# yhenon/pixeltable-yolox

Hardware: AMD Instinct MI355X
Metric: images/sec (fwd+NMS) YOLOX-s 640×640 bf16 @1/2/4/8 MI355X; box mAP parity (higher is better)
Workload: dtype bf16

## Files before the change

### pixeltable-yolox_amd/csrc/conv_ws.hip

```cpp
#include "conv_common.hpp"
#include "lds_dma.hpp"

#ifndef YXH_WS_PROBE
#define YXH_WS_PROBE 0
#endif

#ifndef YXH_WS_PD8
#define YXH_WS_PD8 0
#endif

#ifndef YXH_WS_NPIN
#define YXH_WS_NPIN 48
#endif

#ifndef YXH_WS_ACT_CT
#define YXH_WS_ACT_CT 1
#endif

namespace yxh {

namespace {

template <typename T, int CR>
__device__ __forceinline__ uint4 ws_weight_padk(const ConvParams& p, int n_first, int tap, int kb, int lane) {
    const int frow = lane & 15, fq = lane >> 4;
    const int ch = kb * 32 + fq * 8;
    if (ch >= CR) return make_uint4(0, 0, 0, 0);
    const int n = min(n_first + frow, p.cout - 1);
    return *(const uint4*)((const T*)p.w + ((long long)n * 9 + tap) * CR + ch);
}

__device__ __forceinline__ void pin_agpr(uint4& v) {
    typedef unsigned u32x4v __attribute__((ext_vector_type(4)));
    u32x4v t = {v.x, v.y, v.z, v.w};
    asm volatile("" : "+a"(t));
    v = make_uint4(t.x, t.y, t.z, t.w);
}

constexpr int ws_ps(int c16, int s) {
    return s == 1 ? c16 + (6 - c16 % 4) % 4 : (c16 % 2 ? c16 : c16 + 1);
}
constexpr int ws_hxp(int tx, int s) {
    const int hx = (tx - 1) * s + 3;
    if (tx % 16 == 0) return hx;
    int h = hx;
    while (h % 8 != tx % 8) ++h;
    return h;
}

}

template <typename T, int CIN, int S, int TX, int TY, int TN, int WN, int WK, int WM, int BPC, bool F1, int PGN = 0,
          int PGC = 0, int PGH = 0, int CR = CIN, bool A32 = false>
__global__ __launch_bounds__(64 * WN * WK * WM, BPC) void conv_ws(ConvParams p, int tiles_x, int tiles_y,
                                                                 int ntiles, int ntn, int nwork) {
    static_assert(sizeof(T) == 2, "16-bit operands");
    constexpr int NW = WN * WK * WM;
    constexpr int NCB = CIN / 32, WCB = NCB / WK;
    constexpr int WTN = TN / WN, FR = WTN / 16;
    constexpr int TM = TX * TY, WTM = TM / WM, FC = WTM / 16;
    constexpr int HX = (TX - 1) * S + 3, HY = (TY - 1) * S + 3, HXP = ws_hxp(TX, S);
    constexpr int C16 = CIN / 8, PS = ws_ps(C16, S), PSB = PS * 16;
    constexpr int SLOTS = HY * HXP * PS, LOADS = (SLOTS + 63) / 64, GB = (LOADS + NW - 1) / NW;
    constexpr int RBYTES = WK > 1 ? WN * WM * FR * FC * (WK - 1) * 1024 : 0;
    constexpr bool PG = PGN > 0, HP = PGH > 0, PGY = PG || HP;
    constexpr int RS = TN / 8 + 1, RSLOTS = (S == 1 || PGY) ? TM * RS : 0;
    constexpr int RLOADS = (RSLOTS + 63) / 64, GR = (RLOADS + NW - 1) / NW, RTB = RLOADS * 1024;
    constexpr int NRING = 3;
    constexpr int XS = PGC / 8 + 1, XSLOTS = PG && PGC > 0 ? TM * XS : 0;
    constexpr int XLOADS = (XSLOTS + 63) / 64, GX = (XLOADS + NW - 1) / NW, XTB = XLOADS * 1024;
    constexpr int K2 = TN + PGC, KB2 = K2 / 32;
    constexpr int WN2 = PG ? (NW < PGN / 16 ? NW : PGN / 16) : 1, WM2 = NW / WN2;
    constexpr int NF2 = PG ? PGN / 16 / WN2 : 1, PF2 = TM / 16 / WM2;
    static_assert(!PG || (!F1 && TN % 32 == 0 && PGC % 32 == 0 && PGN % (16 * WN2) == 0 &&
                          NW % WN2 == 0 && (TM / 16) % WM2 == 0), "post-conv tile");
    static_assert(!HP || (!PG && !F1 && S == 1 && TN % 32 == 0), "head-form tile");
    constexpr int HROWS = HP ? PGH * 16 : 0, HBYTES_W = HROWS * RS * 16 + HROWS * 4;
    constexpr int NG = CIN / 32, R1 = NW / NG, NPA = (HY * HXP + 15) / 16;
    constexpr int HBYTES = LOADS * 1024;
    constexpr int XOFF = 2 * HBYTES + RBYTES + NRING * RTB;
    constexpr int TOFF = XOFF + 3 * XTB;
    constexpr int HWOFF = TOFF + (F1 ? HBYTES : 0);
    constexpr int SMEM = HWOFF + HBYTES_W;
    static_assert(!F1 || (S == 1 && NW % NG == 0), "fused Bottleneck tile");
    constexpr int FCO = (FC + WK - 1) / WK;
    constexpr int NS = WCB * 9;
    constexpr int PD = YXH_WS_PD8 && FR * FC >= 8 ? YXH_WS_PD8 : FR * FC >= 8 ? 1 : FR * FC >= 4 ? 2 : 3;
    static_assert(NCB % WK == 0 && WTN % 16 == 0 && WTM % 16 == 0 && TM % (16 * WM) == 0, "tile");
    static_assert(FR * 9 * WCB * 4 <= (NW == 4 && BPC == 1 ? 288 : 160), "weights must stay in VGPRs");
    static_assert(SMEM <= 160 * 1024 && SMEM * BPC <= 160 * 1024, "LDS (BPC blocks per CU must fit)");
    constexpr int NPIN = !F1 && FR * 9 * WCB * 4 > 160 ? YXH_WS_NPIN : 0;
    __shared__ __attribute__((aligned(16))) char smem[SMEM];

    const int tid = threadIdx.x, lane = tid & 63;
    const int wave = __builtin_amdgcn_readfirstlane(tid >> 6);
    const int wn = wave % WN, wk = (wave / WN) % WK, wm = wave / (WN * WK);
    const int frow = lane & 15, fq = lane >> 4;
    const int bid = dma::xcd_remap(blockIdx.x, gridDim.x);
    const int nt = bid % ntn, worker = bid / ntn;
    const int n0 = nt * TN;
    const int tile = worker;
    if (tile >= ntiles) return;

    const int cin_ = p.cin, cout = p.cout, in_w = p.in_w, in_h = p.in_h, scs = p.scs[0];
    const int OH = p.out_h, OW = p.out_w, ohw = p.ohw;
    (void)cin_;

    uint32_t boff[FC];
#pragma unroll
    for (int j = 0; j < FC; ++j) {
        const int pl = (wm * FC + j) * 16 + frow;
        const int ty = pl / TX, tx = pl - ty * TX;
        boff[j] = (uint32_t)((ty * S * HXP + tx * S) * PSB + (wk * WCB * 4 + fq) * 16);
    }

    const uint32_t lds0 = dma::lds_addr(smem);
    const uint32_t bytes = (uint32_t)((long long)in_h * in_w * scs * 2);
    const int gsrc = p.grp2 && n0 >= cout / 2 ? CR : 0;

    int hrel[GB], hyx[GB];
#pragma unroll
    for (int i = 0; i < GB; ++i) {
        const int L = wave + NW * i;
        const int s = 64 * L + lane;
        const int hp = s / PS, c16 = s - hp * PS;
        const int hy = hp / HXP, hx = hp - hy * HXP;
        const bool st = L < LOADS && s < SLOTS && c16 < CR / 8 && hx < HX;
        hyx[i] = st ? (hy | (hx << 16)) : 0x7fff7fff;
        hrel[i] = ((hy * in_w + hx) * scs + c16 * 8) * 2;
    }

    struct TileC { int b, oy0, ox0; };
    const unsigned txy = (unsigned)(tiles_x * tiles_y);
    auto coords = [&](int t) -> TileC {
        const unsigned b = (unsigned)t / txy, r = (unsigned)t - b * txy;
        const unsigned ty = r / (unsigned)tiles_x, tx = r - ty * (unsigned)tiles_x;
        return TileC{(int)b, (int)ty * TY, (int)tx * TX};
    };

    auto issue_halo = [&](const TileC& c, int kb) {
        const int iy0 = c.oy0 * S - 1, ix0 = c.ox0 * S - 1;
        const int base = (iy0 * in_w + ix0) * scs * 2;
        const dma::u32x4 rsrc = dma::srd((const T*)p.sptr[0] + (long long)c.b * p.sbs[0] + gsrc, bytes);
#pragma unroll
        for (int i = 0; i < GB; ++i) {
            const int L = wave + NW * i;
            if (LOADS % NW == 0 || i + 1 < GB || L < LOADS) {
                const int iy = iy0 + (hyx[i] & 0xffff), ix = ix0 + (hyx[i] >> 16);
                const bool ok = (unsigned)iy < (unsigned)in_h && (unsigned)ix < (unsigned)in_w;
                const uint32_t voff = ok ? (uint32_t)(base + hrel[i]) : dma::kOob;
                dma::load16(rsrc, voff, 0u, __builtin_amdgcn_readfirstlane(lds0 + (uint32_t)(kb * HBYTES + L * 1024)));
            }
// ... 339 lines not shown
            for (int j = 0; j < FC; ++j) acc[i][j] = f32x4{0.f, 0.f, 0.f, 0.f};
        const char* hb = F1 ? smem + TOFF : smem + kb * HBYTES;
        uint4 bf[PD + 1][FC];
        auto load_b = [&](int s, uint4 (&d)[FC]) {
            const int c = s / 9, tap = s - 9 * (s / 9);
            const int ky = tap / 3, kx = tap - 3 * (tap / 3);
            const int so = (ky * HXP + kx) * PSB + c * 64;
#pragma unroll
            for (int j = 0; j < FC; ++j) d[j] = *(const uint4*)(hb + boff[j] + so);
        };
#pragma unroll
        for (int q = 0; q < PD; ++q)
            if (q < NS) load_b(q, bf[q]);
        __builtin_amdgcn_sched_group_barrier(0x100, FC * (PD < NS ? PD : NS), 0);
        EpiCtx e{};
        if constexpr (EPI) e = epi_ctx(prev, k - 1);
        PostCtx pc{};
        if constexpr (POST) pc = post_ctx(prev2, k - 2);
        uint4 pob[KBP];
#pragma unroll
        for (int s = 0; s < NS; ++s) {
            if (s + PD < NS) load_b(s + PD, bf[(s + PD) % (PD + 1)]);
            const int c = s / 9, tap = s - 9 * (s / 9);
            if constexpr (FIRST && NPIN > 0) {
#pragma unroll
                for (int i = 0; i < FR; ++i)
                    if ((c * 9 + tap) * FR + i < NPIN) pin_agpr(a[i][tap][c]);
            }
            if constexpr (HP) {
#pragma unroll
                for (int i = 0; i < FR; ++i)
#pragma unroll
                    for (int j = 0; j < FC; ++j) Mma<T>::run(acc[i][j], a[i][tap][c], bf[s % (PD + 1)][j]);
            } else {
#pragma unroll
                for (int j = 0; j < FC; ++j)
#pragma unroll
                    for (int i = 0; i < FR; ++i) Mma<T>::run(acc[i][j], a[i][tap][c], bf[s % (PD + 1)][j]);
            }
            if constexpr (EPI)
                if (s < NP) epi_piece(e, accp, s / FR, s % FR, act_c);
            if constexpr (POST && SPLIT) {
                if (s >= 1 && (s - 1) % SP == 0 && (s - 1) / SP < NPU) post_math(pc, (s - 1) / SP, pob);
                if (s % SP == 0 && s / SP < NPU) post_load(pc, s / SP, pob);
            } else if constexpr (POST) {
                if (s % SP == 0 && s / SP < NPU) post_piece(pc, s / SP);
            }
            if (s + PD < NS) __builtin_amdgcn_sched_group_barrier(0x100, FC, 0);
#pragma unroll
            for (int m = 0; m < FR * FC; ++m) {
                __builtin_amdgcn_sched_group_barrier(0x008, 1, 0);
                if constexpr (EPI) __builtin_amdgcn_sched_group_barrier(0x002, 2, 0);
            }
        }
        if constexpr (EPI)
#pragma unroll
            for (int q = NS; q < NP; ++q) epi_piece(e, accp, q / FR, q % FR, act_c);
        if constexpr (POST) {
            if (SPLIT && (NS - 1) % SP == 0 && (NS - 1) / SP < NPU) post_math(pc, (NS - 1) / SP, pob);
#pragma unroll
            for (int u = (NS + SP - 1) / SP; u < NPU; ++u) post_piece(pc, u);
        }

        if constexpr (WK > 1) {
            char* red = smem + 2 * HBYTES;
            const int grp = wm * WN + wn;
#pragma unroll
            for (int i = 0; i < FR; ++i)
#pragma unroll
                for (int j = 0; j < FC; ++j) {
                    const int own = j % WK;
                    if (own != wk) {
                        const int slot = wk < own ? wk : wk - 1;
                        *(f32x4*)(red + (((grp * FR + i) * FC + j) * (WK - 1) + slot) * 1024 + lane * 16) = acc[i][j];
                    }
                }
            dma::barrier();
#pragma unroll
            for (int i = 0; i < FR; ++i)
#pragma unroll
                for (int j = 0; j < FC; ++j)
                    if (j % WK == wk) {
                        f32x4 v = acc[i][j];
#pragma unroll
                        for (int o = 0; o < WK - 1; ++o)
                            v += *(const f32x4*)(red + (((grp * FR + i) * FC + j) * (WK - 1) + o) * 1024 + lane * 16);
                        accp[i][j / WK] = v;
                    }
        } else {
#pragma unroll
            for (int i = 0; i < FR; ++i)
#pragma unroll
                for (int j = 0; j < FC; ++j) accp[i][j] = acc[i][j];
        }
        return next;
    };

    using act_rt = std::integral_constant<int, 0>;
    int next = tile_step(cur, tile, 0, cnext, cur, cur, std::false_type{}, std::false_type{}, std::true_type{}, act_rt{});
    if constexpr (HP) {
        const T* hw = (const T*)(hgrp1 ? p.pgw2 : p.pgw);
        const float* hb = hgrp1 ? p.pgb2 : p.pgb;
        char* wl = smem + HWOFF;
        for (int q = tid; q < HROWS * (TN / 8); q += 64 * NW) {
            const int r = q / (TN / 8), c = q - (TN / 8) * (q / (TN / 8));
            *(uint4*)(wl + (r * RS + c) * 16) = r < hrows ? *(const uint4*)(hw + (long long)r * TN + c * 8)
                                                          : make_uint4(0, 0, 0, 0);
        }
        for (int q = tid; q < HROWS; q += 64 * NW) ((float*)(wl + HROWS * RS * 16))[q] = q < hrows ? hb[q] : 0.0f;
    }

    constexpr bool ACT_CT = YXH_WS_ACT_CT && !A32 && !PGY && !F1 && NW == 4 && BPC == 1;
    if constexpr (ACT_CT) {
        auto tile_loop = [&](auto act_c) {
            int k = 1;
            for (; next < ntiles; ++k) {
                prev2 = prev;
                prev = cur;
                cur = cnext;
                next = tile_step(cur, next, k, cnext, prev, prev2, std::true_type{}, std::false_type{}, std::false_type{},
                                 act_c);
            }
            epilogue(cur, k - 1, accp, act_c);
        };
        if (silu) tile_loop(std::integral_constant<int, 1>{});
        else tile_loop(std::integral_constant<int, 2>{});
    } else {
        int k = 1;
        for (; next < ntiles; ++k) {
            prev2 = prev;
            prev = cur;
            cur = cnext;
            if (PGY && k >= 2)
                next = tile_step(cur, next, k, cnext, prev, prev2, std::true_type{}, std::integral_constant<bool, PGY>{},
                                 std::false_type{}, act_rt{});
            else
                next = tile_step(cur, next, k, cnext, prev, prev2, std::true_type{}, std::false_type{}, std::false_type{},
                                 act_rt{});
        }
        if constexpr (PGY) {
            dma::wait_vm<0>();
            dma::barrier();
            if (k >= 2) post_all(post_ctx(prev, k - 2));
        }
        epilogue(cur, k - 1, accp, act_rt{});
        if constexpr (PGY) {
            dma::barrier();
            post_all(post_ctx(cur, k - 1));
        }
    }
    (void)ohw;
}

template <typename T, int CIN, int S, int TX, int TY, int TN, int WN, int WK, int WM, int BPC = 1, bool F1 = false,
          int PGN = 0, int PGC = 0, int PGH = 0, int CR = CIN, bool A32 = false>
static int launch_ws(const ConvParams& p, hipStream_t st) {
    if (p.stride != S || p.cin != CR) {
        set_error("conv_ws variant built for stride %d, %d input channels", S, CR);
        return YXH_EUNSUPPORTED;
    }
    if (CR != CIN && (p.grp2 || PGN > 0 || PGH > 0 || F1 || p.scs[0] % 8 || (uintptr_t)p.sptr[0] % 16)) {
        set_error("conv_ws padded-K variant (%d -> %d channels): plain conv over 16-byte pixel rows only", CR, CIN);
        return YXH_EUNSUPPORTED;
    }
    if (PGH > 0) {
        if (!p.grp2 || !p.pgw2 || p.cout != 2 * TN || (p.pg_cout + 15) / 16 != PGH) {
            set_error("conv_ws head-form tile: two groups of %d channels, %d class fragments", TN, PGH);
            return YXH_EUNSUPPORTED;
        }
    } else if ((p.pgw != nullptr) != (PGN > 0) || p.pgw2 || (p.pg_store && PGN == 0) ||
               (PGN > 0 && (p.pg_cout != PGN || p.pgs_ch != PGC || p.cout != TN))) {
        set_error(PGN > 0 ? "conv_ws post tile built for %d -> %d channels + a %d-channel post_src, post conv %d"
                          : "conv_ws plain tile with a post conv (%d -> %d, %d, %d)",
                  CIN, TN, PGC, PGN);
        return YXH_EUNSUPPORTED;
    }
    if (p.grp2 && (F1 || PGN > 0 || (p.cout / 2) % TN)) {
        set_error("conv_ws variant (%d input channels) cannot split its channel tiles over two groups", CIN);
        return YXH_EUNSUPPORTED;
    }
    if ((p.pw1 != nullptr) != F1) {
        set_error(F1 ? "conv_ws fused-Bottleneck variant (%d input channels) needs pre_weight"
                     : "conv_ws plain variant (%d input channels) with a pre_weight",
                  CIN);
        return YXH_EUNSUPPORTED;
    }
    if (A32) {
        if (!p.dst_f32 || p.act != YXH_ACT_NONE || p.res || p.grp2 || p.cout % 4 || ((uintptr_t)p.dst % 16) ||
            p.dst_cs % 4 || p.dst_bs % 4 || (long long)p.ohw * p.dst_cs * 4 >= (1LL << 31)) {
            set_error("conv_ws fp32-gradient tile: fp32 dst of 16-byte rows, no activation / residual");
            return YXH_EUNSUPPORTED;
        }
    } else if (p.dst_f32 || p.accum || (p.act != YXH_ACT_SILU && p.act != YXH_ACT_NONE) ||
        (!p.vec_store && PGN == 0 && PGH == 0) ||
        p.cout % 8 || (p.res && (S != 1 || ((uintptr_t)p.res % 16) || p.res_cs % 8 || p.res_bs % 8))) {
        set_error("conv_ws: 16-bit dst, SiLU/no activation, 8-byte aligned dst rows, 16-byte residual rows "
                  "(stride-1 variants) only");
        return YXH_EUNSUPPORTED;
    }
    const int tiles_x = (p.out_w + TX - 1) / TX, tiles_y = (p.out_h + TY - 1) / TY;
    const long long ntiles = (long long)tiles_x * tiles_y * (p.M / p.ohw);
    const int ntn = (p.cout + TN - 1) / TN;
    if (ntiles >= (1LL << 30)) {
        set_error("conv_ws: too many tiles");
        return YXH_EINVAL;
    }
    const int nwork = (int)std::min<long long>(ntiles, std::max(1, p.cus * BPC / ntn));
    hipLaunchKernelGGL((conv_ws<T, CIN, S, TX, TY, TN, WN, WK, WM, BPC, F1, PGN, PGC, PGH, CR, A32>), dim3((unsigned)(nwork * ntn)),
                       dim3(64 * WN * WK * WM), 0, st, p, tiles_x, tiles_y, (int)ntiles, ntn, nwork);
    YXH_CHECK_LAUNCH("conv_ws launch");
    return YXH_OK;
}

template <typename T>
static int ws_dispatch_t(int id, const ConvParams& p, hipStream_t st) {
    switch (id) {
        case 1: return launch_ws<T, 32, 1, 16, 8, 32, 1, 1, 4>(p, st);
        case 2: return launch_ws<T, 32, 1, 16, 16, 32, 1, 1, 8>(p, st);
        case 3: return launch_ws<T, 32, 2, 16, 8, 64, 2, 1, 4>(p, st);
        case 4: return launch_ws<T, 32, 2, 16, 4, 64, 2, 1, 2, 2>(p, st);
        case 5: return launch_ws<T, 64, 1, 16, 8, 64, 2, 1, 4>(p, st);
        case 6: return launch_ws<T, 64, 1, 16, 4, 64, 2, 1, 2, 2>(p, st);
        case 7: return launch_ws<T, 64, 2, 16, 4, 128, 4, 1, 2>(p, st);
        case 8: return launch_ws<T, 64, 2, 16, 2, 128, 4, 1, 1, 2>(p, st);
        case 11: return launch_ws<T, 128, 1, 8, 4, 128, 4, 2, 1>(p, st);
        case 12: return launch_ws<T, 128, 1, 8, 8, 64, 2, 2, 1>(p, st);
        case 13: return launch_ws<T, 128, 2, 16, 2, 128, 4, 2, 1>(p, st);
        case 14: return launch_ws<T, 128, 2, 8, 4, 128, 4, 2, 1>(p, st);
        case 15: return launch_ws<T, 128, 1, 16, 4, 64, 2, 2, 1>(p, st);
        case 16: return launch_ws<T, 256, 1, 8, 4, 64, 2, 4, 1>(p, st);
        case 17: return launch_ws<T, 256, 1, 16, 2, 64, 2, 4, 1>(p, st);
        case 18: return launch_ws<T, 32, 1, 16, 8, 32, 1, 1, 4, 2>(p, st);
        case 19: return launch_ws<T, 64, 1, 32, 2, 64, 2, 1, 2, 2>(p, st);
        case 20: return launch_ws<T, 128, 1, 16, 2, 64, 2, 2, 1, 2>(p, st);
        case 21: return launch_ws<T, 128, 1, 8, 4, 64, 2, 2, 1, 2>(p, st);
        case 22: return launch_ws<T, 128, 2, 16, 1, 64, 2, 2, 1, 2>(p, st);
        case 23: return launch_ws<T, 256, 1, 8, 2, 32, 1, 4, 1, 2>(p, st);
        case 24: return launch_ws<T, 64, 2, 16, 2, 64, 2, 1, 2, 2>(p, st);
        case 25: return launch_ws<T, 128, 1, 16, 4, 128, 4, 1, 1>(p, st);
        case 26: return launch_ws<T, 128, 1, 16, 2, 128, 4, 1, 1>(p, st);
        case 27: return launch_ws<T, 128, 1, 8, 4, 128, 4, 1, 1>(p, st);
        case 28: return launch_ws<T, 256, 2, 8, 2, 32, 1, 4, 1>(p, st);
        case 29: return launch_ws<T, 256, 2, 8, 2, 64, 2, 4, 1>(p, st);
        case 30: return launch_ws<T, 256, 2, 16, 1, 32, 1, 4, 1>(p, st);
        case 31: return launch_ws<T, 32, 1, 16, 8, 32, 1, 1, 4, 1, true>(p, st);
        case 32: return launch_ws<T, 32, 1, 16, 16, 32, 1, 1, 8, 1, true>(p, st);
        case 33: return launch_ws<T, 64, 1, 16, 4, 64, 2, 1, 2, 1, true>(p, st);
        case 34: return launch_ws<T, 64, 1, 16, 8, 64, 2, 1, 2, 1, true>(p, st);
        case 35: return launch_ws<T, 128, 1, 16, 4, 128, 4, 1, 1, 1, true>(p, st);
        case 36: return launch_ws<T, 128, 1, 8, 4, 128, 4, 1, 1, 1, true>(p, st);
        case 41: return launch_ws<T, 32, 1, 16, 8, 32, 1, 1, 4, 1, false, 64, 32>(p, st);
        case 42: return launch_ws<T, 32, 1, 16, 4, 32, 1, 1, 4, 2, false, 64, 32>(p, st);
        case 43: return launch_ws<T, 64, 1, 16, 4, 64, 2, 1, 2, 1, false, 128, 64>(p, st);
        case 44: return launch_ws<T, 64, 1, 8, 4, 64, 2, 2, 1, 2, false, 128, 64>(p, st);
        case 45: return launch_ws<T, 64, 2, 16, 2, 128, 4, 1, 1, 1, false, 128, 0>(p, st);
        case 46: return launch_ws<T, 64, 2, 16, 4, 128, 4, 1, 1, 1, false, 128, 0>(p, st);
        case 47: return launch_ws<T, 64, 1, 16, 2, 64, 2, 2, 1, 2, false, 128, 64>(p, st);
        case 48: return launch_ws<T, 64, 1, 16, 4, 64, 2, 2, 1, 1, false, 128, 64>(p, st);
        case 49: return launch_ws<T, 64, 2, 16, 2, 128, 4, 2, 1, 1, false, 128, 0>(p, st);
        case 50: return launch_ws<T, 64, 2, 8, 4, 128, 4, 2, 1, 1, false, 128, 0>(p, st);
        case 51: return launch_ws<T, 128, 1, 16, 4, 128, 4, 1, 1, 1, false, 0, 0, 5>(p, st);
        case 53: return launch_ws<T, 128, 1, 16, 2, 128, 4, 1, 1, 1, false, 0, 0, 5>(p, st);
        case 52: return launch_ws<T, 64, 1, 16, 8, 64, 2, 1, 2, 1, false, 64, 0>(p, st);
        case 54: return launch_ws<T, 64, 1, 16, 4, 64, 2, 1, 2, 1, false, 64, 0>(p, st);
        case 55: return launch_ws<T, 128, 1, 8, 4, 128, 4, 1, 1, 1, false, 128, 0>(p, st);
        case 56: return launch_ws<T, 128, 1, 16, 2, 128, 4, 1, 1, 1, false, 128, 0>(p, st);
        case 61: return launch_ws<T, 96, 1, 16, 4, 80, 5, 1, 1, 1, false, 0, 0, 0, 80>(p, st);
        case 62: return launch_ws<T, 96, 1, 16, 4, 32, 2, 1, 2, 2, false, 0, 0, 0, 80>(p, st);
        case 63: return launch_ws<T, 96, 2, 16, 4, 80, 5, 1, 1, 1, false, 0, 0, 0, 80>(p, st);
        case 64: return launch_ws<T, 96, 2, 16, 4, 32, 2, 1, 2, 1, false, 0, 0, 0, 80>(p, st);
        case 65: return launch_ws<T, 160, 1, 16, 4, 64, 4, 1, 1>(p, st);
        case 66: return launch_ws<T, 160, 1, 16, 4, 32, 2, 1, 2>(p, st);
        case 67: return launch_ws<T, 160, 2, 16, 2, 64, 4, 1, 1>(p, st);
        case 68: return launch_ws<T, 160, 2, 16, 2, 32, 2, 1, 2>(p, st);
        case 69: return launch_ws<T, 320, 1, 8, 4, 32, 2, 2, 1>(p, st);
        case 71: return launch_ws<T, 320, 1, 16, 2, 32, 2, 2, 1>(p, st);
        case 72: return launch_ws<T, 320, 2, 16, 1, 32, 2, 2, 1>(p, st);
        case 74: return launch_ws<T, 512, 1, 8, 2, 32, 2, 4, 1>(p, st);
        case 76: return launch_ws<T, 512, 1, 16, 1, 32, 2, 4, 1>(p, st);
        case 79: return launch_ws<T, 160, 1, 16, 2, 64, 4, 1, 1>(p, st);
        case 80: return launch_ws<T, 96, 1, 8, 4, 32, 2, 1, 2, 2, false, 0, 0, 0, 80>(p, st);
        case 81: return launch_ws<T, 96, 1, 16, 4, 32, 2, 1, 2, 2, false, 0, 0, 0, 80, true>(p, st);
        case 82: return launch_ws<T, 160, 1, 16, 4, 64, 4, 1, 1, 1, false, 0, 0, 0, 160, true>(p, st);
        case 83: return launch_ws<T, 160, 1, 16, 4, 32, 2, 1, 2, 1, false, 0, 0, 0, 160, true>(p, st);
        case 84: return launch_ws<T, 320, 1, 8, 4, 32, 2, 2, 1, 1, false, 0, 0, 0, 320, true>(p, st);
        case 85: return launch_ws<T, 320, 1, 16, 2, 32, 2, 2, 1, 1, false, 0, 0, 0, 320, true>(p, st);
        case 86: return launch_ws<T, 64, 1, 16, 4, 64, 2, 1, 2, 2, false, 0, 0, 0, 64, true>(p, st);
        case 87: return launch_ws<T, 128, 1, 16, 4, 128, 4, 1, 1, 1, false, 0, 0, 0, 128, true>(p, st);
        case 88: return launch_ws<T, 256, 1, 8, 4, 64, 2, 4, 1, 1, false, 0, 0, 0, 256, true>(p, st);
        case 89: return launch_ws<T, 32, 1, 16, 4, 80, 5, 1, 1, 1, false, 0, 0, 0, 16>(p, st);
        default: set_error("conv_ws tile id %d", id); return YXH_EINVAL;
    }
}

int conv_ws_dispatch(int dtype, int id, const ConvParams& p, hipStream_t st) {
    if (p.taps != 9 || p.kw != 3 || p.pad != 1 || p.nsrc != 1 || p.sup[0] || p.sw[0] != p.in_w) {
        set_error("conv_ws needs a 3x3 pad-1 conv over one plain source");
        return YXH_EUNSUPPORTED;
    }
    if ((long long)p.in_h * p.in_w * p.scs[0] * 2 >= (1LL << 31)) {
        set_error("conv_ws: image exceeds 31-bit byte offsets");
        return YXH_EUNSUPPORTED;
    }
    if (dtype == YXH_BF16) return ws_dispatch_t<bf16>(id, p, st);
    if (dtype == YXH_F16) return ws_dispatch_t<f16>(id, p, st);
    set_error("conv_ws is built for bf16/f16");
    return YXH_EUNSUPPORTED;
}

}
```

### pixeltable-yolox_amd/csrc/conv_ws1.hip

```cpp
#include "conv_common.hpp"
#include "lds_dma.hpp"

namespace yxh {

template <typename T, int CIN, int TM, int TN, int WN, int WK, int WM, int BPC, int NBUF, bool UP0, bool V16>
__global__ __launch_bounds__(64 * WN * WK * WM, BPC) void conv_ws1(ConvParams p, int ntiles, int ntn, int nwork,
                                                                    int ps, int l0, int l1) {
    static_assert(sizeof(T) == 2, "16-bit operands");
    constexpr int NW = WN * WK * WM;
    constexpr int NCB = CIN / 32, WCB = NCB / WK;
    constexpr int WTN = TN / WN, FR = WTN / 16;
    constexpr int WTM = TM / WM, FC = WTM / 16;
    constexpr int C16 = CIN / 8;
    constexpr int LMAX = (TM * (C16 + 6) + 63) / 64 + 2, GB = (LMAX + NW - 1) / NW, HBYTES = GB * NW * 1024;
    constexpr int RBYTES = WK > 1 ? WN * WM * FR * FC * (WK - 1) * 1024 : 0;
    constexpr int SMEM = NBUF * HBYTES + RBYTES;
    static_assert(NBUF >= 2 && (NBUF - 1) * GB <= 63, "DMA pipeline depth");
    constexpr int FCO = (FC + WK - 1) / WK;
    constexpr int PD = FR * FC >= 8 ? 1 : FR * FC >= 4 ? 2 : 3;
    static_assert(NCB % WK == 0 && WTN % 16 == 0 && WTM % 16 == 0, "tile");
    static_assert(FR * WCB * 4 <= (NW == 4 && BPC == 1 ? 288 : 160), "weights must stay in VGPRs");
    static_assert(SMEM <= 160 * 1024, "LDS");
    __shared__ __attribute__((aligned(16))) char smem[SMEM];

    const int tid = threadIdx.x, lane = tid & 63;
    const int wave = __builtin_amdgcn_readfirstlane(tid >> 6);
    const int wn = wave % WN, wk = (wave / WN) % WK, wm = wave / (WN * WK);
    const int frow = lane & 15, fq = lane >> 4;
    const int bid = dma::xcd_remap(blockIdx.x, gridDim.x);
    const int nt = bid % ntn, worker = bid / ntn;
    const int n0 = nt * TN;
    const int tile = worker;
    if (tile >= ntiles) return;
    const int M = p.M, cout = p.cout, dcs = p.dst_cs;
    const int c0 = p.src0_ch, ncb0 = c0 / 32;
    const int c1 = CIN - c0;

    uint32_t boff[FC];
#pragma unroll
    for (int j = 0; j < FC; ++j) boff[j] = (uint32_t)(((wm * FC + j) * 16 + frow) * ps * 16 + fq * 16);

    int geo[GB];
#pragma unroll
    for (int i = 0; i < GB; ++i) {
        const int L = wave + NW * i;
        const int r = L < l0 ? 0 : 1;
        const int s = 64 * (L - r * l0) + lane;
        const int hp = s / ps, ch = s - hp * ps;
        const bool st = L < l0 + l1 && hp < TM && ch < (r ? c1 : c0) / 8;
        geo[i] = st ? (hp | (ch << 16)) : -1;
    }
    const uint32_t lds0 = dma::lds_addr(smem);
    const long long src0_elems = UP0 ? (long long)(M / p.ohw) * p.sbs[0] : (long long)M * p.scs[0];
    const dma::u32x4 srd0 = dma::srd(p.sptr[0], (uint32_t)(src0_elems * 2));
    const int ohw = p.ohw, ow = p.out_w, sw0 = p.sw[0];
    const long long sbs0 = p.sbs[0];
    const dma::u32x4 srd1 = dma::srd(p.nsrc > 1 ? p.sptr[1] : p.sptr[0],
                                     (uint32_t)((long long)M * (p.nsrc > 1 ? p.scs[1] : p.scs[0]) * 2));
    const int scs0 = p.scs[0], scs1 = p.nsrc > 1 ? p.scs[1] : 0;

    auto issue = [&](int t, int kb) {
        const int m0 = t * TM;
#pragma unroll
        for (int i = 0; i < GB; ++i) {
            const int L = wave + NW * i;
            {
                const int g = geo[i];
                const int m = m0 + (g & 0xffff);
                const bool ok = g >= 0 && m < M;
                const uint32_t ldsa = __builtin_amdgcn_readfirstlane(lds0 + (uint32_t)(kb * HBYTES + L * 1024));
                const bool r0 = L < l0;
                dma::u32x4 rs = r0 ? srd0 : srd1;
                rs.x = __builtin_amdgcn_readfirstlane(rs.x);
                rs.y = __builtin_amdgcn_readfirstlane(rs.y);
                rs.z = __builtin_amdgcn_readfirstlane(rs.z);
                rs.w = __builtin_amdgcn_readfirstlane(rs.w);
                long long e = (long long)m * (r0 ? scs0 : scs1);
                if (UP0 && r0) {
                    const int b = m / ohw, rr = m - b * ohw, y = rr / ow, x = rr - y * ow;
                    e = b * sbs0 + ((long long)(y >> 1) * sw0 + (x >> 1)) * scs0;
                }
                const uint32_t voff = ok ? (uint32_t)((e + (g >> 16) * 8) * 2) : dma::kOob;
                dma::load16(rs, voff, 0u, ldsa);
            }
        }
    };

#pragma unroll
    for (int q = 0; q < NBUF; ++q) issue(tile + q * nwork, q);
    uint4 a[FR][WCB];
#pragma unroll
    for (int c = 0; c < WCB; ++c)
#pragma unroll
        for (int i = 0; i < FR; ++i) a[i][c] = ws_weight<T>(p, n0 + wn * WTN + i * 16, 0, 1, CIN, wk * WCB + c, lane);
    float bias[FR][4];
#pragma unroll
    for (int i = 0; i < FR; ++i) {
        const int n = n0 + wn * WTN + i * 16 + fq * 4;
#pragma unroll
        for (int r = 0; r < 4; ++r) bias[i][r] = n + r < cout ? p.bias[n + r] : 0.0f;
    }

    const bool silu = p.act == YXH_ACT_SILU;
    typedef uint32_t u32x2 __attribute__((ext_vector_type(2)));
    const __amdgpu_buffer_rsrc_t dsrd =
        __builtin_amdgcn_make_buffer_rsrc(p.dst, (short)0, (int)((long long)M * dcs * 2), 0x00020000);
    auto epi_piece = [&](const int tprev, const f32x4 (&ap)[FR][FCO], const int o, const int i) {
        const int j = wk + WK * o;
        const int m = tprev * TM + (wm * FC + j) * 16 + frow;
        const int n = n0 + wn * WTN + i * 16 + fq * 4;
        const bool ok = j < FC && m < M && n < cout;
        const int od = ok ? (m * dcs + n) * 2 : (int)dma::kOob;
        const f32x4 x = ap[i][o] + f32x4{bias[i][0], bias[i][1], bias[i][2], bias[i][3]};
        const f32x4 v = silu ? yxh::silu4(x) : x;
        T t[4] = {from_f32<T>(v[0]), from_f32<T>(v[1]), from_f32<T>(v[2]), from_f32<T>(v[3])};
        u32x2 u;
        __builtin_memcpy(&u, t, 8);
        __builtin_amdgcn_raw_buffer_store_b64(u, dsrd, od, 0, 0);
    };

    auto epi_piece16 = [&](const int tprev, const f32x4 (&ap)[FR][FCO], const int o, const int ip) {
        const int j = wk + WK * o;
        const int i0 = 2 * ip;
        const int m = tprev * TM + (wm * FC + j) * 16 + frow;
        const int n = n0 + wn * WTN + i0 * 16 + (fq & 1) * 16 + (fq >> 1) * 8;
        const bool ok = j < FC && m < M && n < cout;
        const int od = ok ? (m * dcs + n) * 2 : (int)dma::kOob;
        uint32_t w[2][2];
#pragma unroll
        for (int h = 0; h < 2; ++h) {
            const int i = i0 + h;
            const f32x4 x = ap[i][o] + f32x4{bias[i][0], bias[i][1], bias[i][2], bias[i][3]};
            const uint2 pk = pack4<T>(silu ? yxh::silu4(x) : x);
            w[h][0] = pk.x;
            w[h][1] = pk.y;
        }
#pragma unroll
        for (int q = 0; q < 2; ++q) {
            const auto r = __builtin_amdgcn_permlane16_swap(w[0][q], w[1][q], false, false);
            w[0][q] = r[0];
            w[1][q] = r[1];
        }
        typedef uint32_t u32x4 __attribute__((ext_vector_type(4)));
        const u32x4 u = {w[0][0], w[0][1], w[1][0], w[1][1]};
        __builtin_amdgcn_raw_buffer_store_b128(u, dsrd, od, 0, 0);
    };

    f32x4 accp[FR][FCO];
    static_assert(!V16 || FR % 2 == 0, "16-byte epilogue pairs channel fragments");
    constexpr int NP = V16 ? FR / 2 * FCO : FR * FCO;
    constexpr int PFR = V16 ? FR / 2 : FR;
    constexpr int PSP = V16 && 2 * NP <= WCB ? 2 : 1;
    auto piece = [&](const int tprev, const f32x4 (&ap)[FR][FCO], const int q) {
        if constexpr (V16) epi_piece16(tprev, ap, q / PFR, q % PFR);
        else epi_piece(tprev, ap, q / FR, q % FR);
    };
    auto tile_step = [&](const int t, const int k, const int tprev, auto epi, auto first) -> int {
        constexpr bool EPI = decltype(epi)::value;
        constexpr bool FIRST = decltype(first)::value;
        const int kb = k % NBUF;
        const int next = t + nwork;
        if constexpr (FIRST) {
            constexpr int younger = (NBUF - 1) * GB + FR * WCB;
            dma::wait_vm<(younger < 63 ? younger : 63)>();
        } else {
            dma::wait_vm<(NBUF - 2) * GB>();
        }
        dma::barrier();
        if (!FIRST) issue(t + (NBUF - 1) * nwork, (k + NBUF - 1) % NBUF);

        f32x4 acc[FR][FC];
#pragma unroll
        for (int i = 0; i < FR; ++i)
#pragma unroll
            for (int j = 0; j < FC; ++j) acc[i][j] = f32x4{0.f, 0.f, 0.f, 0.f};
        const char* hb = smem + kb * HBYTES;
        uint4 bf[PD + 1][FC];
        auto load_b = [&](int s, uint4 (&d)[FC]) {
            const int cg = wk * WCB + s;
            const int so = cg < ncb0 ? cg * 64 : l0 * 1024 + (cg - ncb0) * 64;
#pragma unroll
            for (int j = 0; j < FC; ++j) d[j] = *(const uint4*)(hb + boff[j] + so);
        };
#pragma unroll
        for (int q = 0; q < PD; ++q)
            if (q < WCB) load_b(q, bf[q]);
        __builtin_amdgcn_sched_group_barrier(0x100, FC * (PD < WCB ? PD : WCB), 0);
#pragma unroll
        for (int s = 0; s < WCB; ++s) {
            if (s + PD < WCB) load_b(s + PD, bf[(s + PD) % (PD + 1)]);
#pragma unroll
            for (int j = 0; j < FC; ++j)
#pragma unroll
                for (int i = 0; i < FR; ++i) Mma<T>::run(acc[i][j], a[i][s], bf[s % (PD + 1)][j]);
            if constexpr (EPI)
                if (s % PSP == 0 && s / PSP < NP) piece(tprev, accp, s / PSP);
            if (s + PD < WCB) __builtin_amdgcn_sched_group_barrier(0x100, FC, 0);
#pragma unroll
            for (int m = 0; m < FR * FC; ++m) {
                __builtin_amdgcn_sched_group_barrier(0x008, 1, 0);
                if constexpr (EPI) __builtin_amdgcn_sched_group_barrier(0x002, 2, 0);
            }
        }
        if constexpr (EPI)
#pragma unroll
            for (int q = (WCB + PSP - 1) / PSP; q < NP; ++q) piece(tprev, accp, q);

        if constexpr (WK > 1) {
            char* red = smem + NBUF * HBYTES;
            const int grp = wm * WN + wn;
#pragma unroll
            for (int i = 0; i < FR; ++i)
#pragma unroll
                for (int j = 0; j < FC; ++j) {
                    const int own = j % WK;
                    if (own != wk) {
                        const int slot = wk < own ? wk : wk - 1;
                        *(f32x4*)(red + (((grp * FR + i) * FC + j) * (WK - 1) + slot) * 1024 + lane * 16) = acc[i][j];
                    }
                }
            dma::barrier();
#pragma unroll
            for (int i = 0; i < FR; ++i)
#pragma unroll
                for (int j = 0; j < FC; ++j)
                    if (j % WK == wk) {
                        f32x4 v = acc[i][j];
#pragma unroll
                        for (int o = 0; o < WK - 1; ++o)
                            v += *(const f32x4*)(red + (((grp * FR + i) * FC + j) * (WK - 1) + o) * 1024 + lane * 16);
                        accp[i][j / WK] = v;
                    }
        } else {
#pragma unroll
            for (int i = 0; i < FR; ++i)
#pragma unroll
                for (int j = 0; j < FC; ++j) accp[i][j] = acc[i][j];
        }
        return next;
    };

    int cur = tile;
    int next = tile_step(cur, 0, 0, std::false_type{}, std::true_type{});
    int k = 1;
    for (; next < ntiles; ++k) {
        const int prev = cur;
        cur = next;
        next = tile_step(cur, k, prev, std::true_type{}, std::false_type{});
    }
#pragma unroll
    for (int q = 0; q < NP; ++q) piece(cur, accp, q);
    dma::wait_vm<0>();
}

template <typename T, int CIN, int TM, int TN, int WN, int WK, int WM, int BPC = 1, int NBUF = 2, bool UP0 = false>
static int launch_ws1(const ConvParams& p, hipStream_t st) {
    if (p.cin != CIN) {
        set_error("conv_ws1 variant built for %d input channels", CIN);
        return YXH_EUNSUPPORTED;
    }
    const int c0 = p.src0_ch, c1 = CIN - c0;
    const bool srcs_ok = UP0 ? (p.nsrc == 2 && p.sup[0] == 1 && p.sup[1] == 0 && p.sw[0] * 2 == p.out_w &&
                                p.sw[1] == p.out_w && p.sbs[1] == (long long)p.ohw * p.scs[1] &&
                                (long long)(p.M / p.ohw) * p.sbs[0] * 2 < (1LL << 31))
                             : (bool)p.src_dense;
    if (!srcs_ok || !p.dst_dense || p.dst_f32 || p.accum || p.res || p.pw1 || p.grp2 ||
        (p.act != YXH_ACT_SILU && p.act != YXH_ACT_NONE) || p.cout % 8 || c0 % 32 || c1 % 32 ||
        (p.nsrc == 1) != (c1 == 0)) {
        set_error("conv_ws1: dense 1x1 over 32-channel-aligned sources, 16-bit dst, SiLU/no activation, %d input channels",
                  CIN);
        return YXH_EUNSUPPORTED;
    }
    const long long M = p.M;
    if (M * p.scs[0] * 2 >= (1LL << 31) || (p.nsrc > 1 && M * p.scs[1] * 2 >= (1LL << 31)) ||
        M * p.dst_cs * 2 >= (1LL << 31)) {
        set_error("conv_ws1: tensors exceed 31-bit byte offsets");
        return YXH_EUNSUPPORTED;
    }
    int ps = std::max(c0, c1) / 8;
    ps += (6 - ps % 4) % 4;
    const int l0 = (TM * ps + 63) / 64, l1 = c1 ? (TM * ps + 63) / 64 : 0;
    if (l0 + l1 > (TM * (CIN / 8 + 6) + 63) / 64 + 2) {
        set_error("conv_ws1: source split %d + %d does not fit the LDS image", c0, c1);
        return YXH_EUNSUPPORTED;
    }
    const long long ntiles = (M + TM - 1) / TM;
    const int ntn = (p.cout + TN - 1) / TN;
    const int nwork = (int)std::min<long long>(ntiles, std::max(1, p.cus * BPC / ntn));
    constexpr bool PAIRS = (TN / WN / 16) % 2 == 0;
    if (p.v16_req && !PAIRS) {
        set_error("conv_ws1 tile has no 16-byte epilogue (an odd number of channel fragments per wave)");
        return YXH_EUNSUPPORTED;
    }
    if (PAIRS && p.v16_req && p.vec16)
        hipLaunchKernelGGL((conv_ws1<T, CIN, TM, TN, WN, WK, WM, BPC, NBUF, UP0, PAIRS>), dim3((unsigned)(nwork * ntn)),
                           dim3(64 * WN * WK * WM), 0, st, p, (int)ntiles, ntn, nwork, ps, l0, l1);
    else
        hipLaunchKernelGGL((conv_ws1<T, CIN, TM, TN, WN, WK, WM, BPC, NBUF, UP0, false>), dim3((unsigned)(nwork * ntn)),
                           dim3(64 * WN * WK * WM), 0, st, p, (int)ntiles, ntn, nwork, ps, l0, l1);
    YXH_CHECK_LAUNCH("conv_ws1 launch");
    return YXH_OK;
}

template <typename T>
static int ws1_dispatch_t(int id, const ConvParams& p, hipStream_t st) {
    switch (id) {
        case 1: return launch_ws1<T, 64, 128, 64, 2, 1, 2, 2>(p, st);
        case 2: return launch_ws1<T, 64, 256, 64, 2, 1, 4, 1>(p, st);
        case 3: return launch_ws1<T, 128, 64, 128, 4, 1, 1, 2>(p, st);
        case 4: return launch_ws1<T, 128, 128, 64, 2, 1, 2, 1>(p, st);
        case 5: return launch_ws1<T, 256, 64, 128, 4, 1, 1, 2>(p, st);
        case 6: return launch_ws1<T, 256, 64, 64, 2, 1, 2, 2>(p, st);
        case 7: return launch_ws1<T, 512, 32, 128, 4, 1, 1, 1>(p, st);
        case 8: return launch_ws1<T, 512, 64, 64, 2, 2, 2, 1>(p, st);
        case 9: return launch_ws1<T, 1024, 32, 64, 2, 2, 2, 1>(p, st);
        case 10: return launch_ws1<T, 256, 128, 128, 4, 1, 2, 1>(p, st);
        case 11: return launch_ws1<T, 64, 64, 64, 2, 1, 2, 2, 4>(p, st);
        case 12: return launch_ws1<T, 128, 64, 128, 4, 1, 1, 1, 4>(p, st);
        case 13: return launch_ws1<T, 256, 32, 128, 4, 1, 1, 1, 4>(p, st);
        case 14: return launch_ws1<T, 256, 64, 128, 4, 1, 1, 1, 3>(p, st);
        case 15: return launch_ws1<T, 512, 32, 128, 4, 1, 1, 1, 3>(p, st);
        case 16: return launch_ws1<T, 512, 32, 64, 2, 2, 2, 1, 3>(p, st);
        case 17: return launch_ws1<T, 1024, 16, 64, 4, 1, 1, 1, 4>(p, st);
        case 18: return launch_ws1<T, 64, 128, 64, 2, 1, 2, 1, 3>(p, st);
        case 19: return launch_ws1<T, 512, 32, 128, 4, 1, 1, 1, 3, true>(p, st);
        case 20: return launch_ws1<T, 512, 64, 64, 2, 2, 2, 1, 2, true>(p, st);
        case 21: return launch_ws1<T, 256, 64, 128, 4, 1, 1, 2, 2, true>(p, st);
        case 22: return launch_ws1<T, 256, 32, 128, 4, 1, 1, 1, 4, true>(p, st);
        case 23: return launch_ws1<T, 256, 32, 256, 4, 1, 1, 1, 3>(p, st);
        case 24: return launch_ws1<T, 256, 64, 256, 4, 1, 1, 1, 3>(p, st);
        case 25: return launch_ws1<T, 512, 16, 256, 4, 2, 1, 1, 4>(p, st);
        case 26: return launch_ws1<T, 512, 16, 256, 4, 2, 1, 1, 4, true>(p, st);
        case 27: return launch_ws1<T, 128, 64, 256, 4, 1, 1, 1, 3>(p, st);
        case 28: return launch_ws1<T, 1024, 32, 128, 4, 2, 1, 1, 2>(p, st);
        default: set_error("conv_ws1 tile id %d", id); return YXH_EINVAL;
    }
}

int conv_ws1_dispatch(int dtype, int id, const ConvParams& p, hipStream_t st) {
    if (p.taps != 1 || p.stride != 1 || p.pad != 0) {
        set_error("conv_ws1 needs a 1x1 s1 conv");
        return YXH_EUNSUPPORTED;
    }
    if (dtype == YXH_BF16) return ws1_dispatch_t<bf16>(id, p, st);
    if (dtype == YXH_F16) return ws1_dispatch_t<f16>(id, p, st);
    set_error("conv_ws1 is built for bf16/f16");
    return YXH_EUNSUPPORTED;
}

}
```

Measured before the change: 19840.

## Balance 1x1 conv tail tiles across workers and add fallback tile for conv_ws

The 1x1 conv kernel now gives each worker only full tiles in its main loop. Leftover rows are split into 16-row fragments spread evenly over all workers and computed in a short-tile path, so the last wave of work no longer lands on a few workers. Global offsets are also precomputed per lane to trim address math. Separately, one spatial conv variant switches to a 4x4 pixel tile when the output width does not divide its 8-wide tile. Both paths are on by default and can be turned off with environment variables. They add code paths and an extra barrier, and raise register pressure.

Measured after the change: 19950, median of 6. Within noise of the previous version (+0.5%).

```diff
diff --git a/pixeltable-yolox_amd/csrc/conv_ws.hip b/pixeltable-yolox_amd/csrc/conv_ws.hip
--- a/pixeltable-yolox_amd/csrc/conv_ws.hip
+++ b/pixeltable-yolox_amd/csrc/conv_ws.hip
@@ -1,3 +1,5 @@
+#include <cstdlib>
+
 #include "conv_common.hpp"
 #include "lds_dma.hpp"
 
@@ -643,9 +645,17 @@
     (void)ohw;
 }
 
+static bool ws_fit() {
+    const char* e = getenv("YOLOX_AMD_WS_FIT");
+    return !(e && e[0] == '0' && e[1] == 0);
+}
+
 template <typename T, int CIN, int S, int TX, int TY, int TN, int WN, int WK, int WM, int BPC = 1, bool F1 = false,
-          int PGN = 0, int PGC = 0, int PGH = 0, int CR = CIN, bool A32 = false>
+          int PGN = 0, int PGC = 0, int PGH = 0, int CR = CIN, bool A32 = false, int FTX = 0, int FTY = 0>
 static int launch_ws(const ConvParams& p, hipStream_t st) {
+    if constexpr (FTX > 0)
+        if (p.stride == S && p.out_w % TX != 0 && p.out_w % FTX == 0 && ws_fit())
+            return launch_ws<T, CIN, S, FTX, FTY, TN, WN, WK, WM, BPC, F1, PGN, PGC, PGH, CR, A32>(p, st);
     if (p.stride != S || p.cin != CR) {
         set_error("conv_ws variant built for stride %d, %d input channels", S, CR);
         return YXH_EUNSUPPORTED;
@@ -732,7 +742,7 @@
         case 26: return launch_ws<T, 128, 1, 16, 2, 128, 4, 1, 1>(p, st);
         case 27: return launch_ws<T, 128, 1, 8, 4, 128, 4, 1, 1>(p, st);
         case 28: return launch_ws<T, 256, 2, 8, 2, 32, 1, 4, 1>(p, st);
-        case 29: return launch_ws<T, 256, 2, 8, 2, 64, 2, 4, 1>(p, st);
+        case 29: return launch_ws<T, 256, 2, 8, 2, 64, 2, 4, 1, 1, false, 0, 0, 0, 256, false, 4, 4>(p, st);
         case 30: return launch_ws<T, 256, 2, 16, 1, 32, 1, 4, 1>(p, st);
         case 31: return launch_ws<T, 32, 1, 16, 8, 32, 1, 1, 4, 1, true>(p, st);
         case 32: return launch_ws<T, 32, 1, 16, 16, 32, 1, 1, 8, 1, true>(p, st);
diff --git a/pixeltable-yolox_amd/csrc/conv_ws1.hip b/pixeltable-yolox_amd/csrc/conv_ws1.hip
--- a/pixeltable-yolox_amd/csrc/conv_ws1.hip
+++ b/pixeltable-yolox_amd/csrc/conv_ws1.hip
@@ -1,11 +1,14 @@
+#include <cstdlib>
+
 #include "conv_common.hpp"
 #include "lds_dma.hpp"
+#include "tile_partition.hpp"
 
 namespace yxh {
 
 template <typename T, int CIN, int TM, int TN, int WN, int WK, int WM, int BPC, int NBUF, bool UP0, bool V16>
-__global__ __launch_bounds__(64 * WN * WK * WM, BPC) void conv_ws1(ConvParams p, int ntiles, int ntn, int nwork,
-                                                                    int ps, int l0, int l1) {
+__global__ __launch_bounds__(64 * WN * WK * WM, BPC) void conv_ws1(ConvParams p, int ntn, int nwork, int ps, int l0,
+                                                                    int l1, int tail) {
     static_assert(sizeof(T) == 2, "16-bit operands");
     constexpr int NW = WN * WK * WM;
     constexpr int NCB = CIN / 32, WCB = NCB / WK;
@@ -30,9 +33,12 @@
     const int bid = dma::xcd_remap(blockIdx.x, gridDim.x);
     const int nt = bid % ntn, worker = bid / ntn;
     const int n0 = nt * TN;
-    const int tile = worker;
-    if (tile >= ntiles) return;
     const int M = p.M, cout = p.cout, dcs = p.dst_cs;
+    constexpr bool TAILS = TM > kTileFrag;
+    const TilePartition part = tile_partition(M, TM, nwork, worker, TAILS && tail != 0);
+    const int R = part.rounds, sm0 = TAILS ? part.tail_m0 : 0, sm1 = TAILS ? part.tail_m1 : 0;
+    const bool has_tail = TAILS && sm1 > sm0;
+    if (R == 0) return;
     const int c0 = p.src0_ch, ncb0 = c0 / 32;
     const int c1 = CIN - c0;
 
@@ -58,16 +64,22 @@
     const dma::u32x4 srd1 = dma::srd(p.nsrc > 1 ? p.sptr[1] : p.sptr[0],
                                      (uint32_t)((long long)M * (p.nsrc > 1 ? p.scs[1] : p.scs[0]) * 2));
     const int scs0 = p.scs[0], scs1 = p.nsrc > 1 ? p.scs[1] : 0;
-
-    auto issue = [&](int t, int kb) {
-        const int m0 = t * TM;
+    uint32_t goff[GB];
+#pragma unroll
+    for (int i = 0; i < GB; ++i)
+        goff[i] = (uint32_t)(((geo[i] & 0xffff) * (wave + NW * i < l0 ? scs0 : scs1) + (geo[i] >> 16) * 8) * 2);
+
+    auto issue = [&](int q, int kb) {
+        const int m0 = q < R ? (worker + q * nwork) * TM : sm0;
+        const int mlim = q < R ? M : q == R ? sm1 : 0;
+        const uint32_t base0 = (uint32_t)m0 * (uint32_t)scs0 * 2u, base1 = (uint32_t)m0 * (uint32_t)scs1 * 2u;
 #pragma unroll
         for (int i = 0; i < GB; ++i) {
             const int L = wave + NW * i;
             {
                 const int g = geo[i];
                 const int m = m0 + (g & 0xffff);
-                const bool ok = g >= 0 && m < M;
+                const bool ok = g >= 0 && m < mlim;
                 const uint32_t ldsa = __builtin_amdgcn_readfirstlane(lds0 + (uint32_t)(kb * HBYTES + L * 1024));
                 const bool r0 = L < l0;
                 dma::u32x4 rs = r0 ? srd0 : srd1;
@@ -75,19 +87,20 @@
                 rs.y = __builtin_amdgcn_readfirstlane(rs.y);
                 rs.z = __builtin_amdgcn_readfirstlane(rs.z);
                 rs.w = __builtin_amdgcn_readfirstlane(rs.w);
-                long long e = (long long)m * (r0 ? scs0 : scs1);
+                uint32_t off = (r0 ? base0 : base1) + goff[i];
                 if (UP0 && r0) {
                     const int b = m / ohw, rr = m - b * ohw, y = rr / ow, x = rr - y * ow;
-                    e = b * sbs0 + ((long long)(y >> 1) * sw0 + (x >> 1)) * scs0;
+                    const long long e = b * sbs0 + ((long long)(y >> 1) * sw0 + (x >> 1)) * scs0;
+                    off = (uint32_t)((e + (g >> 16) * 8) * 2);
                 }
-                const uint32_t voff = ok ? (uint32_t)((e + (g >> 16) * 8) * 2) : dma::kOob;
+                const uint32_t voff = ok ? off : dma::kOob;
                 dma::load16(rs, voff, 0u, ldsa);
             }
         }
     };
 
 #pragma unroll
-    for (int q = 0; q < NBUF; ++q) issue(tile + q * nwork, q);
+    for (int q = 0; q < NBUF; ++q) issue(q, q);
     uint4 a[FR][WCB];
 #pragma unroll
     for (int c = 0; c < WCB; ++c)
@@ -105,11 +118,11 @@
     typedef uint32_t u32x2 __attribute__((ext_vector_type(2)));
     const __amdgpu_buffer_rsrc_t dsrd =
         __builtin_amdgcn_make_buffer_rsrc(p.dst, (short)0, (int)((long long)M * dcs * 2), 0x00020000);
-    auto epi_piece = [&](const int tprev, const f32x4 (&ap)[FR][FCO], const int o, const int i) {
+    auto epi_piece = [&](const int mb, const int ml, const f32x4 (&ap)[FR][FCO], const int o, const int i) {
         const int j = wk + WK * o;
-        const int m = tprev * TM + (wm * FC + j) * 16 + frow;
+        const int m = mb + (wm * FC + j) * 16 + frow;
         const int n = n0 + wn * WTN + i * 16 + fq * 4;
-        const bool ok = j < FC && m < M && n < cout;
+        const bool ok = j < FC && m < ml && n < cout;
         const int od = ok ? (m * dcs + n) * 2 : (int)dma::kOob;
         const f32x4 x = ap[i][o] + f32x4{bias[i][0], bias[i][1], bias[i][2], bias[i][3]};
         const f32x4 v = silu ? yxh::silu4(x) : x;
@@ -119,12 +132,12 @@
         __builtin_amdgcn_raw_buffer_store_b64(u, dsrd, od, 0, 0);
     };
 
-    auto epi_piece16 = [&](const int tprev, const f32x4 (&ap)[FR][FCO], const int o, const int ip) {
+    auto epi_piece16 = [&](const int mb, const int ml, const f32x4 (&ap)[FR][FCO], const int o, const int ip) {
         const int j = wk + WK * o;
         const int i0 = 2 * ip;
-        const int m = tprev * TM + (wm * FC + j) * 16 + frow;
+        const int m = mb + (wm * FC + j) * 16 + frow;
         const int n = n0 + wn * WTN + i0 * 16 + (fq & 1) * 16 + (fq >> 1) * 8;
-        const bool ok = j < FC && m < M && n < cout;
+        const bool ok = j < FC && m < ml && n < cout;
         const int od = ok ? (m * dcs + n) * 2 : (int)dma::kOob;
         uint32_t w[2][2];
 #pragma unroll
@@ -151,15 +164,18 @@
     constexpr int NP = V16 ? FR / 2 * FCO : FR * FCO;
     constexpr int PFR = V16 ? FR / 2 : FR;
     constexpr int PSP = V16 && 2 * NP <= WCB ? 2 : 1;
-    auto piece = [&](const int tprev, const f32x4 (&ap)[FR][FCO], const int q) {
-        if constexpr (V16) epi_piece16(tprev, ap, q / PFR, q % PFR);
-        else epi_piece(tprev, ap, q / FR, q % FR);
-    };
-    auto tile_step = [&](const int t, const int k, const int tprev, auto epi, auto first) -> int {
+    auto piece = [&](const int mb, const int ml, const f32x4 (&ap)[FR][FCO], const int q) {
+        if constexpr (V16) epi_piece16(mb, ml, ap, q / PFR, q % PFR);
+        else epi_piece(mb, ml, ap, q / FR, q % FR);
+    };
+    auto red_slot = [&](char* red, const int i, const int j, const int slot) {
+        return (f32x4*)(red + ((((wm * WN + wn) * FR + i) * FC + j) * (WK - 1) + slot) * 1024 + lane * 16);
+    };
+    auto tile_step = [&](const int k, auto epi, auto first) {
         constexpr bool EPI = decltype(epi)::value;
         constexpr bool FIRST = decltype(first)::value;
         const int kb = k % NBUF;
-        const int next = t + nwork;
+        const int mprev = (worker + (k - 1) * nwork) * TM;
         if constexpr (FIRST) {
             constexpr int younger = (NBUF - 1) * GB + FR * WCB;
             dma::wait_vm<(younger < 63 ? younger : 63)>();
@@ -167,7 +183,7 @@
             dma::wait_vm<(NBUF - 2) * GB>();
         }
         dma::barrier();
-        if (!FIRST) issue(t + (NBUF - 1) * nwork, (k + NBUF - 1) % NBUF);
+        if (!FIRST) issue(k + NBUF - 1, (k + NBUF - 1) % NBUF);
 
         f32x4 acc[FR][FC];
 #pragma unroll
@@ -194,7 +210,7 @@
 #pragma unroll
                 for (int i = 0; i < FR; ++i) Mma<T>::run(acc[i][j], a[i][s], bf[s % (PD + 1)][j]);
             if constexpr (EPI)
-                if (s % PSP == 0 && s / PSP < NP) piece(tprev, accp, s / PSP);
+                if (s % PSP == 0 && s / PSP < NP) piece(mprev, M, accp, s / PSP);
             if (s + PD < WCB) __builtin_amdgcn_sched_group_barrier(0x100, FC, 0);
 #pragma unroll
             for (int m = 0; m < FR * FC; ++m) {
@@ -204,20 +220,16 @@
         }
         if constexpr (EPI)
 #pragma unroll
-            for (int q = (WCB + PSP - 1) / PSP; q < NP; ++q) piece(tprev, accp, q);
+            for (int q = (WCB + PSP - 1) / PSP; q < NP; ++q) piece(mprev, M, accp, q);
 
         if constexpr (WK > 1) {
             char* red = smem + NBUF * HBYTES;
-            const int grp = wm * WN + wn;
 #pragma unroll
             for (int i = 0; i < FR; ++i)
 #pragma unroll
                 for (int j = 0; j < FC; ++j) {
                     const int own = j % WK;
-                    if (own != wk) {
-                        const int slot = wk < own ? wk : wk - 1;
-                        *(f32x4*)(red + (((grp * FR + i) * FC + j) * (WK - 1) + slot) * 1024 + lane * 16) = acc[i][j];
-                    }
+                    if (own != wk) *red_slot(red, i, j, wk < own ? wk : wk - 1) = acc[i][j];
                 }
             dma::barrier();
 #pragma unroll
@@ -227,8 +239,7 @@
                     if (j % WK == wk) {
                         f32x4 v = acc[i][j];
 #pragma unroll
-                        for (int o = 0; o < WK - 1; ++o)
-                            v += *(const f32x4*)(red + (((grp * FR + i) * FC + j) * (WK - 1) + o) * 1024 + lane * 16);
+                        for (int o = 0; o < WK - 1; ++o) v += *red_slot(red, i, j, o);
                         accp[i][j / WK] = v;
                     }
         } else {
@@ -237,20 +248,82 @@
 #pragma unroll
                 for (int j = 0; j < FC; ++j) accp[i][j] = acc[i][j];
         }
-        return next;
-    };
-
-    int cur = tile;
-    int next = tile_step(cur, 0, 0, std::false_type{}, std::true_type{});
-    int k = 1;
-    for (; next < ntiles; ++k) {
-        const int prev = cur;
-        cur = next;
-        next = tile_step(cur, k, prev, std::true_type{}, std::false_type{});
-    }
-#pragma unroll
-    for (int q = 0; q < NP; ++q) piece(cur, accp, q);
+    };
+
+    auto short_tile = [&] {
+        const int nfw = (sm1 - sm0 + 15) / 16 - wm * FC;
+        const char* hb = smem + (R % NBUF) * HBYTES;
+        f32x4 acc[FR][FC];
+#pragma unroll
+        for (int j = 0; j < FC; ++j) {
+#pragma unroll
+            for (int i = 0; i < FR; ++i) acc[i][j] = f32x4{0.f, 0.f, 0.f, 0.f};
+            if (j < nfw) {
+                constexpr int TPD = WCB < 8 ? WCB : 8;
+                uint4 b[TPD];
+                auto load_b = [&](int s) {
+                    const int cg = wk * WCB + s;
+                    const int so = cg < ncb0 ? cg * 64 : l0 * 1024 + (cg - ncb0) * 64;
+                    return *(const uint4*)(hb + boff[j] + so);
+                };
+#pragma unroll
+                for (int s = 0; s < TPD; ++s) b[s] = load_b(s);
+#pragma unroll
+                for (int s = 0; s < WCB; ++s) {
+                    const uint4 bs = b[s % TPD];
+                    if (s + TPD < WCB) b[s % TPD] = load_b(s + TPD);
+#pragma unroll
+                    for (int i = 0; i < FR; ++i) Mma<T>::run(acc[i][j], a[i][s], bs);
+                }
+            }
+        }
+        if constexpr (WK > 1) {
+            char* red = smem + NBUF * HBYTES;
+#pragma unroll
+            for (int i = 0; i < FR; ++i)
+#pragma unroll
+                for (int j = 0; j < FC; ++j) {
+                    const int own = j % WK;
+                    if (own != wk && j < nfw) *red_slot(red, i, j, wk < own ? wk : wk - 1) = acc[i][j];
+                }
+            dma::barrier();
+#pragma unroll
+            for (int i = 0; i < FR; ++i)
+#pragma unroll
+                for (int j = 0; j < FC; ++j)
+                    if (j % WK == wk) {
+                        f32x4 v = acc[i][j];
+                        if (j < nfw)
+#pragma unroll
+                            for (int o = 0; o < WK - 1; ++o) v += *red_slot(red, i, j, o);
+                        accp[i][j / WK] = v;
+                    }
+        } else {
+#pragma unroll
+            for (int i = 0; i < FR; ++i)
+#pragma unroll
+                for (int j = 0; j < FC; ++j) accp[i][j] = acc[i][j];
+        }
+#pragma unroll
+        for (int q = 0; q < NP; ++q)
+            if (wk + WK * (q / PFR) < nfw) piece(sm0, sm1, accp, q);
+    };
+    tile_step(0, std::false_type{}, std::true_type{});
+    for (int k = 1; k < R; ++k) tile_step(k, std::true_type{}, std::false_type{});
+    if (has_tail) {
+        dma::wait_vm<(NBUF - 2) * GB>();
+        dma::barrier();
+    }
+    const int mlast = (worker + (R - 1) * nwork) * TM;
+#pragma unroll
+    for (int q = 0; q < NP; ++q) piece(mlast, M, accp, q);
+    if (has_tail) short_tile();
     dma::wait_vm<0>();
+}
+
+static bool ws1_tail() {
+    const char* e = getenv("YOLOX_AMD_WS1_TAIL");
+    return !(e && e[0] == '0' && e[1] == 0);
 }
 
 template <typename T, int CIN, int TM, int TN, int WN, int WK, int WM, int BPC = 1, int NBUF = 2, bool UP0 = false>
@@ -287,6 +360,7 @@
     const long long ntiles = (M + TM - 1) / TM;
     const int ntn = (p.cout + TN - 1) / TN;
     const int nwork = (int)std::min<long long>(ntiles, std::max(1, p.cus * BPC / ntn));
+    const int tail = ws1_tail() && TM > kTileFrag;
     constexpr bool PAIRS = (TN / WN / 16) % 2 == 0;
     if (p.v16_req && !PAIRS) {
         set_error("conv_ws1 tile has no 16-byte epilogue (an odd number of channel fragments per wave)");
@@ -294,10 +368,10 @@
     }
     if (PAIRS && p.v16_req && p.vec16)
         hipLaunchKernelGGL((conv_ws1<T, CIN, TM, TN, WN, WK, WM, BPC, NBUF, UP0, PAIRS>), dim3((unsigned)(nwork * ntn)),
-                           dim3(64 * WN * WK * WM), 0, st, p, (int)ntiles, ntn, nwork, ps, l0, l1);
+                           dim3(64 * WN * WK * WM), 0, st, p, ntn, nwork, ps, l0, l1, tail);
     else
         hipLaunchKernelGGL((conv_ws1<T, CIN, TM, TN, WN, WK, WM, BPC, NBUF, UP0, false>), dim3((unsigned)(nwork * ntn)),
-                           dim3(64 * WN * WK * WM), 0, st, p, (int)ntiles, ntn, nwork, ps, l0, l1);
+                           dim3(64 * WN * WK * WM), 0, st, p, ntn, nwork, ps, l0, l1, tail);
     YXH_CHECK_LAUNCH("conv_ws1 launch");
     return YXH_OK;
 }
diff --git a/pixeltable-yolox_amd/csrc/tile_partition.hpp b/pixeltable-yolox_amd/csrc/tile_partition.hpp
--- /dev/null
+++ b/pixeltable-yolox_amd/csrc/tile_partition.hpp
@@ -0,0 +1,39 @@
+#pragma once
+
+#if defined(__HIPCC__) || defined(__CUDACC__)
+#define YXH_TP_HD __host__ __device__ inline
+#else
+#define YXH_TP_HD inline
+#endif
+
+namespace yxh {
+
+constexpr int kTileFrag = 16;
+
+struct TilePartition {
+    int rounds;
+    int tail_m0;
+    int tail_m1;
+};
+
+YXH_TP_HD TilePartition tile_partition(int M, int TM, int nwork, int w, bool tail) {
+    TilePartition r;
+    if (!tail || (M / TM) / nwork == 0) {
+        const int ntiles = (M + TM - 1) / TM;
+        r.rounds = w < ntiles ? (ntiles - w + nwork - 1) / nwork : 0;
+        r.tail_m0 = r.tail_m1 = 0;
+        return r;
+    }
+    r.rounds = (M / TM) / nwork;
+    const int left0 = r.rounds * nwork * TM;
+    const int nfrag = (M - left0 + kTileFrag - 1) / kTileFrag;
+    const int q = nfrag / nwork, rem = nfrag % nwork;
+    const int f0 = w * q + (w < rem ? w : rem);
+    const int f1 = f0 + q + (w < rem ? 1 : 0);
+    const int m0 = left0 + f0 * kTileFrag, m1 = left0 + f1 * kTileFrag;
+    r.tail_m0 = m0 < M ? m0 : M;
+    r.tail_m1 = m1 < M ? m1 : M;
+    return r;
+}
+
+}
```
